# yangbang18/CARE

Hardware: AMD Instinct MI355X
Metric: captions/sec (greedy) (higher is better)
Workload: dtype bf16; 1 GPU; MSRVTT Transformer/base task=Base feats=ViT modality=ami greedy (BASELINE.json configs[1]): [B,28,128]+[B,28,2048]+[B,28,512] fp32 feats, d=512, V=10547, 29 decoder steps; config_name=msrvtt_base_ami, global_batch=32768, lanes=1, parallelism=batch-sharded dp1 (no data-path collective; all-gather of results), hip_graph=True, absorbed_cross_attention=True, lean_encode=True

## Files before the change

care_amd/csrc/gemm_ln.hip:

```cpp
#include <cstdlib>
#include <type_traits>

#include "care_common.h"

namespace {

constexpr int LN_N = 512;

struct LnArgs {
  const void* A; int64_t lda;
  const bf16_t* W;
  const float* bias; const float* res; int64_t ldres; const float* pos;
  const float* gamma; const float* beta; float eps;
  float* out; bf16_t* outb; int64_t ldo;
  int M, K, grp, out_grp_rows, out_row_off;
  int w_packed;
};

template <int N>
__device__ __forceinline__ void ln_wait_vm() {
  if constexpr (N == 5) asm volatile("s_waitcnt vmcnt(5)" ::: "memory");
  else if constexpr (N == 6) asm volatile("s_waitcnt vmcnt(6)" ::: "memory");
  else if constexpr (N == 9) asm volatile("s_waitcnt vmcnt(9)" ::: "memory");
  else if constexpr (N == 10) asm volatile("s_waitcnt vmcnt(10)" ::: "memory");
  else asm volatile("s_waitcnt vmcnt(0)" ::: "memory");
}

template <bool AF32, int RG>
__global__ __launch_bounds__(256 * RG, RG == 1 ? 1 : 2) void gemm_ln_kernel(LnArgs p) {
  constexpr int BM = 64 * RG, NW = 4 * RG;
  constexpr int A_ROWB = AF32 ? 128 : 64;
  constexpr int A_BYTES = BM * A_ROWB, W_BYTES = LN_N * 64, SLOT = A_BYTES + W_BYTES;
  constexpr int NA = A_BYTES / 1024, NWI = W_BYTES / 1024;
  constexpr int NPW = (NA + NWI) / NW;
  static_assert((NA + NWI) % NW == 0, "DMA instructions must divide evenly over the waves");
  extern __shared__ __attribute__((aligned(16))) unsigned char smem[];

  const int tid = threadIdx.x, lane = tid & 63;
  const int wave = __builtin_amdgcn_readfirstlane(tid >> 6);
  const int rg = wave >> 2, cg = wave & 3;
  const int fr = lane & 15, fg = lane >> 4;
  const int m0 = blockIdx.x * BM;
  constexpr unsigned HTAB = (2u) | (3u << 3) | (4u << 6) | (2u << 9) | (5u << 12) | (7u << 15) | (4u << 18) | (1u << 21);

  const unsigned char* src[NPW];
  int dst_off[NPW];
#pragma unroll
  for (int i = 0; i < NPW; ++i) {
    const int q = wave * NPW + i;
    if (q < NA) {
      if constexpr (AF32) {
        const int row = q * 8 + (lane >> 3), pch = lane & 7;
        const int ch = pch ^ ((HTAB >> (3 * ((row & 15) >> 1))) & 7);
        const int grow = min(m0 + row, p.M - 1);
        src[i] = reinterpret_cast<const unsigned char*>(reinterpret_cast<const float*>(p.A) + (int64_t)grow * p.lda) + ch * 16;
      } else {
        const int row = q * 16 + (lane >> 2), pch = lane & 3;
        const int ch = pch ^ ((row & 8) >> 2);
        const int grow = min(m0 + row, p.M - 1);
        src[i] = reinterpret_cast<const unsigned char*>(reinterpret_cast<const bf16_t*>(p.A) + (int64_t)grow * p.lda) + ch * 16;
      }
      dst_off[i] = q * 1024;
    } else {
      const int n = (q - NA) * 16 + (lane >> 2), pch = lane & 3;
      const int ch = pch ^ ((n & 8) >> 2);
      src[i] = reinterpret_cast<const unsigned char*>(p.W + (int64_t)n * p.K) + ch * 16;
      dst_off[i] = A_BYTES + (q - NA) * 1024;
    }
  }
  auto stage = [&](int kt, int slot) {
#pragma unroll
    for (int i = 0; i < NPW; ++i) {
      const int q = wave * NPW + i;
      const int step = (q < NA) ? A_ROWB : 64;
      __builtin_amdgcn_global_load_lds((const __attribute__((address_space(1))) void*)(src[i] + (int64_t)kt * step),
                                       (__attribute__((address_space(3))) void*)(smem + slot * SLOT + dst_off[i]),
                                       16, 0, 0);
    }
  };

  f32x4 acc[4][8];
#pragma unroll
  for (int mt = 0; mt < 4; ++mt)
#pragma unroll
    for (int nt = 0; nt < 8; ++nt) acc[mt][nt] = f32x4{0.f, 0.f, 0.f, 0.f};

  int a_off[4][AF32 ? 2 : 1], w_off[8];
#pragma unroll
  for (int mt = 0; mt < 4; ++mt) {
    const int row = rg * 64 + mt * 16 + fr;
    if constexpr (AF32) {
      const int x = (HTAB >> (3 * (fr >> 1))) & 7;
      a_off[mt][0] = row * 128 + (((2 * fg) ^ x) << 4);
      a_off[mt][1] = row * 128 + (((2 * fg + 1) ^ x) << 4);
    } else {
      a_off[mt][0] = row * 64 + ((fg ^ ((fr & 8) >> 2)) << 4);
    }
  }
#pragma unroll
  for (int nt = 0; nt < 8; ++nt) w_off[nt] = A_BYTES + (cg * 128 + nt * 16 + fr) * 64 + ((fg ^ ((fr & 8) >> 2)) << 4);

  const int nk = p.K >> 5;
  stage(0, 0);
  if (nk > 1) stage(1, 1);
  __builtin_amdgcn_sched_barrier(0);

  for (int kt = 0; kt < nk; ++kt) {
    if (kt + 1 < nk) ln_wait_vm<NPW>(); else ln_wait_vm<0>();
    __builtin_amdgcn_s_barrier();
    __builtin_amdgcn_sched_barrier(0);
    if (kt + 2 < nk) stage(kt + 2, (kt + 2) % 3);
    __builtin_amdgcn_sched_barrier(0);
    const unsigned char* sl = smem + (kt % 3) * SLOT;
    bf16x8 fa[4], fb[8];
#pragma unroll
    for (int nt = 0; nt < 8; ++nt) fb[nt] = *reinterpret_cast<const bf16x8*>(sl + w_off[nt]);
#pragma unroll
    for (int mt = 0; mt < 4; ++mt) {
      if constexpr (AF32) {
        const float4 lo = *reinterpret_cast<const float4*>(sl + a_off[mt][0]);
        const float4 hi = *reinterpret_cast<const float4*>(sl + a_off[mt][1]);
        fa[mt][0] = (bf16_t)lo.x; fa[mt][1] = (bf16_t)lo.y; fa[mt][2] = (bf16_t)lo.z; fa[mt][3] = (bf16_t)lo.w;
        fa[mt][4] = (bf16_t)hi.x; fa[mt][5] = (bf16_t)hi.y; fa[mt][6] = (bf16_t)hi.z; fa[mt][7] = (bf16_t)hi.w;
      } else {
        fa[mt] = *reinterpret_cast<const bf16x8*>(sl + a_off[mt][0]);
      }
    }
#pragma unroll
    for (int mt = 0; mt < 4; ++mt)
#pragma unroll
      for (int nt = 0; nt < 8; ++nt)
        acc[mt][nt] = care_mfma_16x16x32_h16(fb[nt], fa[mt], acc[mt][nt], 0, 0, 0);
  }

  float* tile = reinterpret_cast<float*>(smem);
  float4 gm[2], bt[2], bs[2];
#pragma unroll
  for (int h = 0; h < 2; ++h) {
    const int col = (h * 64 + lane) * 4;
    gm[h] = *reinterpret_cast<const float4*>(p.gamma + col);
    bt[h] = *reinterpret_cast<const float4*>(p.beta + col);
    bs[h] = p.bias ? *reinterpret_cast<const float4*>(p.bias + col) : make_float4(0.f, 0.f, 0.f, 0.f);
  }
#pragma unroll 1
  for (int g = 0; g < RG; ++g) {
    __syncthreads();
    if (rg == g) {
#pragma unroll
      for (int mt = 0; mt < 4; ++mt)
#pragma unroll
        for (int nt = 0; nt < 8; ++nt) {
          const int row = mt * 16 + fr;
          const int chunk = (cg * 32 + nt * 4 + fg) ^ fr;
          *reinterpret_cast<f32x4*>(tile + row * LN_N + chunk * 4) = acc[mt][nt];
        }
    }
    __syncthreads();
    constexpr int UNR = 4, RPW = 64 / NW;
#pragma unroll 1
    for (int rb = 0; rb < RPW; rb += UNR) {
      float4 v[UNR][2], rs[UNR][2], ps[UNR][2];
      int grow[UNR];
#pragma unroll
      for (int u = 0; u < UNR; ++u) {
        const int r = wave * RPW + rb + u;
        grow[u] = m0 + g * 64 + r;
        const int gc = min(grow[u], p.M - 1);
#pragma unroll
        for (int h = 0; h < 2; ++h) {
          const int chunk = h * 64 + lane;
          v[u][h] = *reinterpret_cast<const float4*>(tile + r * LN_N + ((chunk ^ (r & 15)) * 4));
          if (p.res) rs[u][h] = *reinterpret_cast<const float4*>(p.res + (int64_t)gc * p.ldres + chunk * 4);
          if (p.pos) ps[u][h] = *reinterpret_cast<const float4*>(p.pos + (int64_t)(gc % p.grp) * LN_N + chunk * 4);
        }
      }
#pragma unroll
      for (int u = 0; u < UNR; ++u) {
        if (grow[u] >= p.M) continue;
#pragma unroll
        for (int h = 0; h < 2; ++h) {
          v[u][h].x += bs[h].x; v[u][h].y += bs[h].y; v[u][h].z += bs[h].z; v[u][h].w += bs[h].w;
          if (p.res) { v[u][h].x += rs[u][h].x; v[u][h].y += rs[u][h].y; v[u][h].z += rs[u][h].z; v[u][h].w += rs[u][h].w; }
          if (p.pos) { v[u][h].x += ps[u][h].x; v[u][h].y += ps[u][h].y; v[u][h].z += ps[u][h].z; v[u][h].w += ps[u][h].w; }
        }
        const float s = ((v[u][0].x + v[u][0].y) + (v[u][0].z + v[u][0].w)) + ((v[u][1].x + v[u][1].y) + (v[u][1].z + v[u][1].w));
        const float mean = care_wave_sum(s) * (1.0f / LN_N);
        float q = 0.f;
#pragma unroll
        for (int h = 0; h < 2; ++h) {
          const float a = v[u][h].x - mean, b = v[u][h].y - mean, c = v[u][h].z - mean, e = v[u][h].w - mean;
          q += (a * a + b * b) + (c * c + e * e);
        }
        const float rstd = 1.0f / sqrtf(care_wave_sum(q) * (1.0f / LN_N) + p.eps);
        const int64_t orow = (int64_t)(grow[u] / p.grp) * p.out_grp_rows + p.out_row_off + (grow[u] % p.grp);
#pragma unroll
        for (int h = 0; h < 2; ++h) {
          const int col = (h * 64 + lane) * 4;
          float4 o;
          o.x = (v[u][h].x - mean) * rstd * gm[h].x + bt[h].x;
          o.y = (v[u][h].y - mean) * rstd * gm[h].y + bt[h].y;
          o.z = (v[u][h].z - mean) * rstd * gm[h].z + bt[h].z;
          o.w = (v[u][h].w - mean) * rstd * gm[h].w + bt[h].w;
          if (p.out) *reinterpret_cast<float4*>(p.out + orow * p.ldo + col) = o;
          if (p.outb) {
            bf16x4 ob;
            ob[0] = (bf16_t)o.x; ob[1] = (bf16_t)o.y; ob[2] = (bf16_t)o.z; ob[3] = (bf16_t)o.w;
            *reinterpret_cast<bf16x4*>(p.outb + orow * p.ldo + col) = ob;
          }
        }
      }
    }
  }
}

template <bool AF32, int RG>
int launch_ln(const LnArgs& p, hipStream_t st) {
  constexpr int BM = 64 * RG;
  constexpr size_t ring = 3 * (BM * (AF32 ? 128 : 64) + LN_N * 64);
  constexpr size_t lds = ring > 64 * LN_N * 4 ? ring : 64 * LN_N * 4;
  const int blocks = (p.M + BM - 1) / BM;
  static std::atomic<unsigned long long> lds_ok{0};
  if (const int e = care_allow_dynamic_lds(reinterpret_cast<const void*>(&gemm_ln_kernel<AF32, RG>), (int)lds, lds_ok)) return e;
  hipLaunchKernelGGL((gemm_ln_kernel<AF32, RG>), dim3(blocks), dim3(256 * RG), lds, st, p);
  return care_launch_status();
}


#ifndef CARE_LN_ST_NT
#define CARE_LN_ST_NT 0
#endif
#ifndef CARE_LN_A_AUX
#define CARE_LN_A_AUX 0
#endif
#ifndef CARE_LN_DBG
#define CARE_LN_DBG 0
#endif
template <bool F16>
__device__ __forceinline__ f32x4 ln2_mfma(const bf16x8& b, const bf16x8& a, const f32x4& c) {
  if constexpr (F16) {
    typedef _Float16 f16x8 __attribute__((ext_vector_type(8)));
    return __builtin_amdgcn_mfma_f32_16x16x32_f16(__builtin_bit_cast(f16x8, b), __builtin_bit_cast(f16x8, a), c, 0, 0, 0);
  } else {
    return care_mfma_16x16x32_h16(b, a, c, 0, 0, 0);
  }
}

template <int N>
__device__ __forceinline__ void ln2_wait_vm() {
  static_assert(N >= 0 && N <= 63, "vmcnt immediate");
  asm volatile("s_waitcnt vmcnt(%0)" ::"n"(N) : "memory");
}

template <int PER, int MAXY>
__device__ __forceinline__ void ln2_wait_stages(int younger) {
  static_assert(MAXY * PER <= 63, "vmcnt range");
  if constexpr (MAXY >= 6) { if (younger >= 6) { ln2_wait_vm<6 * PER>(); return; } }
  if constexpr (MAXY >= 5) { if (younger == 5) { ln2_wait_vm<5 * PER>(); return; } }
  if constexpr (MAXY >= 4) { if (younger == 4) { ln2_wait_vm<4 * PER>(); return; } }
  if constexpr (MAXY >= 3) { if (younger == 3) { ln2_wait_vm<3 * PER>(); return; } }
  if constexpr (MAXY >= 2) { if (younger == 2) { ln2_wait_vm<2 * PER>(); return; } }
  if constexpr (MAXY >= 1) { if (younger == 1) { ln2_wait_vm<PER>(); return; } }
  ln2_wait_vm<0>();
}

template <bool AF32, int RG, int NSW, int NSA, int EPI, int REP = 1>
__global__ __launch_bounds__(256 * RG, RG) void gemm_ln2_kernel(LnArgs p) {
  static_assert(REP == 1 || (REP == 3 && AF32), "split products need the fp32 operand");
  constexpr int BM = 64 * RG, NW = 4 * RG, NLD = NW / 2;
  constexpr int A_ROWB = 256, KSUB = AF32 ? 2 : 4;
  constexpr int A_BYTES = BM * A_ROWB, W_BYTES = LN_N * 64;
  constexpr int A_BASE = NSW * W_BYTES;
  constexpr int NWI = W_BYTES / 1024 / NLD;
  constexpr int NAI = A_BYTES / 1024 / NLD;
  static_assert(NSW >= 2 && NSA >= 2, "ring depths");
  constexpr bool AE = NSA == 2;
  static_assert(!AE || (!AF32 && REP == 1), "early A issue: bf16 A only");
  extern __shared__ __attribute__((aligned(16))) unsigned char smem[];

  const int tid = threadIdx.x, lane = tid & 63;
  const int wave = __builtin_amdgcn_readfirstlane(tid >> 6);
  const int rg = wave >> 2, cg = wave & 3;
  const int fr = lane & 15, fg = lane >> 4;
  const int m0 = blockIdx.x * BM;
  const bool w_loader = wave < NLD;
  constexpr unsigned HTAB = (2u) | (3u << 3) | (4u << 6) | (2u << 9) | (5u << 12) | (7u << 15) | (4u << 18) | (1u << 21);

  const unsigned w_lane = p.w_packed ? (unsigned)lane * 16u
                                     : (unsigned)(lane >> 2) * (unsigned)p.K * 2u + (unsigned)(((lane & 3) ^ (((lane >> 2) & 8) >> 2)) << 4);
  unsigned a_src[NAI];
#pragma unroll
  for (int i = 0; i < NAI; ++i) {
    const int row = ((w_loader ? 0 : wave - NLD) * NAI + i) * 4 + (lane >> 4);
    const int ch = (lane & 15) ^ (row & 15);
    a_src[i] = (unsigned)(min(m0 + row, p.M - 1) - m0) * (unsigned)p.lda * (AF32 ? 4u : 2u) + (unsigned)ch * 16u;
  }
  const unsigned char* a_blk = reinterpret_cast<const unsigned char*>(p.A) + (int64_t)m0 * p.lda * (AF32 ? 4 : 2);
  auto dma_w = [&](int kt, int slot, int i) {
    if (CARE_LN_DBG & 2) return;
    const int q = wave * NWI + i;
    const unsigned char* base = reinterpret_cast<const unsigned char*>(p.W) +
                                (p.w_packed ? (int64_t)kt * W_BYTES + q * 1024 : (int64_t)(q * 16) * p.K * 2 + (int64_t)kt * 64);
    __builtin_amdgcn_global_load_lds((const __attribute__((address_space(1))) void*)(base + w_lane),
                                     (__attribute__((address_space(3))) void*)(smem + (slot % NSW) * W_BYTES + q * 1024),
                                     16, 0, 0);
  };
  auto dma_a = [&](int m, int slot, int i) {
    if (CARE_LN_DBG & 4) return;
    __builtin_amdgcn_global_load_lds((const __attribute__((address_space(1))) void*)(a_blk + (int64_t)m * A_ROWB + a_src[i]),
                                     (__attribute__((address_space(3))) void*)(smem + A_BASE + (slot % NSA) * A_BYTES + ((wave - NLD) * NAI + i) * 1024),
                                     16, 0, CARE_LN_A_AUX);
  };

  f32x4 acc[4][8];
#pragma unroll
  for (int mt = 0; mt < 4; ++mt)
#pragma unroll
    for (int nt = 0; nt < 8; ++nt) acc[mt][nt] = f32x4{0.f, 0.f, 0.f, 0.f};

  const int w_off0 = (cg * 128 + 8 * (fr >> 2) + (fr & 3)) * 64 + ((fg ^ ((fr & 4) >> 1)) << 4);
  const int a_lane = A_BASE + (rg * 64 + fr) * A_ROWB + (((AF32 ? 2 * fg : fg) ^ fr) << 4);
  auto read_b = [&](int kt, int h, bf16x8 (&f)[4]) {
    if (CARE_LN_DBG & 8) { for (int q = 0; q < 4; ++q) { f[q] = bf16x8{}; asm volatile("" : "+v"(f[q])); } return; }
    const unsigned char* sw = smem + (kt % NSW) * W_BYTES + w_off0;
#pragma unroll
    for (int q = 0; q < 4; ++q) {
      const int nt = h * 4 + q;
      f[q] = *reinterpret_cast<const bf16x8*>(sw + ((nt >> 1) * 32 + (nt & 1) * 4) * 64);
    }
  };
  using araw_t = typename std::conditional<AF32, f32x4, bf16x8>::type;
  auto read_a = [&](int kt, int part, araw_t (&r)[2][AF32 ? 2 : 1]) {
    if (CARE_LN_DBG & 8) { for (int t = 0; t < 2; ++t) for (int c = 0; c < (AF32 ? 2 : 1); ++c) { r[t][c] = araw_t{}; asm volatile("" : "+v"(r[t][c])); } return; }
    const int kr = kt / REP;
    const int jx = (kr % KSUB) * (AF32 ? 128 : 64);
    const unsigned char* sa = smem + ((kr / KSUB) % NSA) * A_BYTES + (a_lane ^ jx);
    const unsigned char* sx = smem + ((kr / KSUB) % NSA) * A_BYTES + (a_lane ^ jx ^ 16);
#pragma unroll
    for (int t = 0; t < 2; ++t) {
      r[t][0] = *reinterpret_cast<const araw_t*>(sa + (2 * part + t) * 16 * A_ROWB);
      if constexpr (AF32) r[t][1] = *reinterpret_cast<const araw_t*>(sx + (2 * part + t) * 16 * A_ROWB);
    }
  };
  auto cvt_a = [&](const araw_t (&r)[2][AF32 ? 2 : 1], bf16x8 (&f)[4], int part, int kt) {
    const bool lo = REP == 3 && kt % REP == 2;
#pragma unroll
    for (int t = 0; t < 2; ++t) {
      if constexpr (AF32) {
        typedef float f32x2 __attribute__((ext_vector_type(2)));
        typedef h16_t bf16x2 __attribute__((ext_vector_type(2)));
        if constexpr (REP == 3) {
          typedef _Float16 f16x2 __attribute__((ext_vector_type(2)));
          typedef unsigned u32x4v __attribute__((ext_vector_type(4)));
          u32x4v packed;
#pragma unroll
          for (int c = 0; c < 2; ++c)
#pragma unroll
            for (int e = 0; e < 4; e += 2) {
              f16x2 pr = __builtin_convertvector(f32x2{r[t][c][e], r[t][c][e + 1]}, f16x2);
              if (lo) pr = __builtin_convertvector(f32x2{r[t][c][e] - (float)pr[0], r[t][c][e + 1] - (float)pr[1]}, f16x2);
              packed[2 * c + (e >> 1)] = __builtin_bit_cast(unsigned, pr);
            }
          f[2 * part + t] = __builtin_bit_cast(bf16x8, packed);
        } else {
#pragma unroll
          for (int c = 0; c < 2; ++c)
#pragma unroll
            for (int e = 0; e < 4; e += 2) {
              bf16x2 pr = __builtin_convertvector(f32x2{r[t][c][e], r[t][c][e + 1]}, bf16x2);
              f[2 * part + t][4 * c + e] = pr[0]; f[2 * part + t][4 * c + e + 1] = pr[1];
            }
        }
      } else {
        f[2 * part + t] = r[t][0];
      }
    }
  };

  const int nk = (p.K >> 5) * REP, nmac = (p.K >> 5) / KSUB;
  constexpr int NAS = NAI / KSUB;
  static_assert(NAI % KSUB == 0 && 16 % NAI == 0, "A issue schedule");
  if (w_loader) {
#pragma unroll 1
    for (int s = 0; s < NSW; ++s)
#pragma unroll
      for (int i = 0; i < NWI; ++i) dma_w(min(s, nk - 1), s, i);
    ln2_wait_vm<(NSW - 1) * NWI>();
  } else {
#pragma unroll 1
    for (int s = 0; s < NSA - 1; ++s)
#pragma unroll
      for (int i = 0; i < NAI; ++i) dma_a(min(s, nmac - 1), s, i);
    ln2_wait_vm<(NSA - 2) * NAI>();
  }
  __builtin_amdgcn_s_barrier();
  __builtin_amdgcn_sched_barrier(0);

  bf16x8 faA[4], fbA[4], faB[4], fbB[4];
  {
    araw_t r0[2][AF32 ? 2 : 1], r1[2][AF32 ? 2 : 1];
    read_a(0, 0, r0); read_a(0, 1, r1); read_b(0, 0, fbA);
    cvt_a(r0, faA, 0, 0); cvt_a(r1, faA, 1, 0);
  }
  auto kstep = [&](int kt, bf16x8 (&fa)[4], bf16x8 (&fb0)[4], bf16x8 (&fan)[4], bf16x8 (&fbn)[4]) {
    const bool more = kt + 1 < nk;
    const int kr = kt / REP, mode = kt % REP;
    const int mac = kr / KSUB, sub = kr % KSUB;
    const bool a_issue = mode == 0;
    const bool a_edge = sub == KSUB - 1 && mode == REP - 1;
    bf16x8 fb1[4];
    araw_t ra[2][AF32 ? 2 : 1], rb[2][AF32 ? 2 : 1];
    __builtin_amdgcn_sched_barrier(0);
    read_b(kt, 1, fb1);
    __builtin_amdgcn_sched_barrier(0);
#pragma unroll
    for (int mt = 0; mt < 4; ++mt)
#pragma unroll
      for (int q = 0; q < 4; ++q)
        if (CARE_LN_DBG & 1) asm volatile("" :: "v"(fb0[q]), "v"(fa[mt]));
        else acc[mt][q] = ln2_mfma<REP == 3>(fb0[q], fa[mt], acc[mt][q]);
    __builtin_amdgcn_sched_barrier(0);
    if (more) {
      if (w_loader) ln2_wait_vm<(NSW - 2) * NWI>();
      else if (a_edge) ln2_wait_vm<AE ? 0 : REP == 1 ? (NSA - 3) * NAI + (KSUB - 1) * NAS : (NSA - 2) * NAI>();
      asm volatile("s_waitcnt lgkmcnt(0)" ::: "memory");
      __builtin_amdgcn_s_barrier();
      __builtin_amdgcn_sched_barrier(0);
      read_a(kt + 1, 0, ra);
      read_b(kt + 1, 0, fbn);
    }
    __builtin_amdgcn_sched_barrier(0);
    const int wst = min(kt + NSW, nk - 1), wslot = kt + NSW;
    const int ast = min(mac - 1 + NSA, nmac - 1), aslot = mac - 1 + NSA;
#pragma unroll
    for (int mt = 0; mt < 4; ++mt) {
#pragma unroll
      for (int q = 0; q < 4; ++q) {
        if (CARE_LN_DBG & 1) asm volatile("" :: "v"(fb1[q]), "v"(fa[mt]));
        else acc[mt][4 + q] = ln2_mfma<REP == 3>(fb1[q], fa[mt], acc[mt][4 + q]);
        const int m = mt * 4 + q;
        if ((m + 1) % (16 / NWI) == 0 || (m + 1) % (16 / (AE ? NAI : NAS)) == 0) {
          if (w_loader) { if ((m + 1) % (16 / NWI) == 0) dma_w(wst, wslot, m / (16 / NWI)); }
          else if (AE) { if (sub == 0 && (m + 1) % (16 / NAI) == 0) dma_a(ast, aslot, m / (16 / NAI)); }
          else { if (a_issue && (m + 1) % (16 / NAS) == 0) dma_a(ast, aslot, sub * NAS + m / (16 / NAS)); }
        }
        __builtin_amdgcn_sched_barrier(0);
      }
      if (mt == 1 && more) {
        cvt_a(ra, fan, 0, kt + 1);
        read_a(kt + 1, 1, rb);
        __builtin_amdgcn_sched_barrier(0);
      }
    }
    if (more) cvt_a(rb, fan, 1, kt + 1);
  };

#pragma unroll 1
  for (int kt = 0; kt < nk; kt += 2) {
    kstep(kt, faA, fbA, faB, fbB);
    kstep(kt + 1, faB, fbB, faA, fbA);
  }

  asm volatile("s_waitcnt vmcnt(0) lgkmcnt(0)" ::: "memory");
  __builtin_amdgcn_s_barrier();
  if (CARE_LN_DBG & 16) {
    float s = 0.f;
#pragma unroll
    for (int mt = 0; mt < 4; ++mt)
#pragma unroll
      for (int nt = 0; nt < 8; ++nt) s += acc[mt][nt][0] + acc[mt][nt][1] + acc[mt][nt][2] + acc[mt][nt][3];
    if (s == 12345.678f && p.outb) p.outb[0] = (bf16_t)s;
    return;
  }
  float* stat = reinterpret_cast<float*>(smem);
  const int col0 = cg * 128 + 8 * fg;
  int m0e = m0;
  asm volatile("" : "+s"(m0e));
  int grow[4];
#pragma unroll
  for (int mt = 0; mt < 4; ++mt) grow[mt] = m0e + rg * 64 + mt * 16 + fr;

  float rsum[4] = {0.f, 0.f, 0.f, 0.f};
  {
    int dep = 0;
    int64_t roff[4], poff[4];
#pragma unroll
    for (int mt = 0; mt < 4; ++mt) {
      const int gc = min(grow[mt], p.M - 1);
      roff[mt] = (int64_t)gc * p.ldres;
      poff[mt] = (int64_t)(gc % p.grp) * LN_N;
    }
#pragma unroll
    for (int pq = 0; pq < 4; ++pq) {
      const int c = col0 + 32 * pq;
      float4 b0 = make_float4(0.f, 0.f, 0.f, 0.f), b1 = b0;
      if (p.bias) { b0 = *reinterpret_cast<const float4*>(p.bias + c); b1 = *reinterpret_cast<const float4*>(p.bias + c + 4); }
      float4 r[4][2], q[4][2];
#pragma unroll
      for (int mth = 0; mth < 2; ++mth) {
#pragma unroll
      for (int mt = 2 * mth; mt < 2 * mth + 2; ++mt) {
        if constexpr (EPI == 1) {
          r[mt][0] = *reinterpret_cast<const float4*>(p.res + roff[mt] + c + dep);
          r[mt][1] = *reinterpret_cast<const float4*>(p.res + roff[mt] + c + 4 + dep);
        }
        if constexpr (EPI == 2) {
          q[mt][0] = *reinterpret_cast<const float4*>(p.pos + poff[mt] + c);
          q[mt][1] = *reinterpret_cast<const float4*>(p.pos + poff[mt] + c + 4);
        }
      }
#pragma unroll
      for (int mt = 2 * mth; mt < 2 * mth + 2; ++mt) {
        f32x4& v0 = acc[mt][2 * pq];
        f32x4& v1 = acc[mt][2 * pq + 1];
        v0[0] += b0.x; v0[1] += b0.y; v0[2] += b0.z; v0[3] += b0.w;
        v1[0] += b1.x; v1[1] += b1.y; v1[2] += b1.z; v1[3] += b1.w;
        if constexpr (EPI == 1) {
          v0[0] += r[mt][0].x; v0[1] += r[mt][0].y; v0[2] += r[mt][0].z; v0[3] += r[mt][0].w;
          v1[0] += r[mt][1].x; v1[1] += r[mt][1].y; v1[2] += r[mt][1].z; v1[3] += r[mt][1].w;
        }
        if constexpr (EPI == 2) {
          v0[0] += q[mt][0].x; v0[1] += q[mt][0].y; v0[2] += q[mt][0].z; v0[3] += q[mt][0].w;
          v1[0] += q[mt][1].x; v1[1] += q[mt][1].y; v1[2] += q[mt][1].z; v1[3] += q[mt][1].w;
        }
        rsum[mt] += ((v0[0] + v0[1]) + (v0[2] + v0[3])) + ((v1[0] + v1[1]) + (v1[2] + v1[3]));
      }
      asm volatile("" : "+v"(dep) : "v"(rsum[2 * mth]), "v"(rsum[2 * mth + 1]));
      __builtin_amdgcn_sched_barrier(0);
      }
    }
  }
  float mean[4], rstd[4];
#pragma unroll
  for (int mt = 0; mt < 4; ++mt) {
    float s = rsum[mt];
    s += __shfl_xor(s, 16, 64);
    s += __shfl_xor(s, 32, 64);
    if (fg == 0) stat[(rg * 64 + mt * 16 + fr) * 4 + cg] = s;
  }
  __syncthreads();
#pragma unroll
  for (int mt = 0; mt < 4; ++mt) {
    const float4 t = *reinterpret_cast<const float4*>(stat + (rg * 64 + mt * 16 + fr) * 4);
    mean[mt] = ((t.x + t.y) + (t.z + t.w)) * (1.0f / LN_N);
  }
#pragma unroll
  for (int mt = 0; mt < 4; ++mt) {
    float q = 0.f;
#pragma unroll
    for (int nt = 0; nt < 8; ++nt) {
      const float a = acc[mt][nt][0] - mean[mt], b = acc[mt][nt][1] - mean[mt];
      const float c = acc[mt][nt][2] - mean[mt], e = acc[mt][nt][3] - mean[mt];
      q += (a * a + b * b) + (c * c + e * e);
    }
    q += __shfl_xor(q, 16, 64);
    q += __shfl_xor(q, 32, 64);
    if (fg == 0) stat[BM * 4 + (rg * 64 + mt * 16 + fr) * 4 + cg] = q;
  }
  __syncthreads();
  int64_t orow[4];
#pragma unroll
  for (int mt = 0; mt < 4; ++mt) {
    const float4 t = *reinterpret_cast<const float4*>(stat + BM * 4 + (rg * 64 + mt * 16 + fr) * 4);
    rstd[mt] = 1.0f / sqrtf(((t.x + t.y) + (t.z + t.w)) * (1.0f / LN_N) + p.eps);
    orow[mt] = (int64_t)(grow[mt] / p.grp) * p.out_grp_rows + p.out_row_off + (grow[mt] % p.grp);
  }
  const float* gam = p.gamma;
  const float* bet = p.beta;
  asm volatile("" : "+s"(gam), "+s"(bet));
#pragma unroll
  for (int pq = 0; pq < 4; ++pq) {
    const int c = col0 + 32 * pq;
    const float4 g0 = *reinterpret_cast<const float4*>(gam + c), g1 = *reinterpret_cast<const float4*>(gam + c + 4);
    const float4 e0 = *reinterpret_cast<const float4*>(bet + c), e1 = *reinterpret_cast<const float4*>(bet + c + 4);
#pragma unroll
    for (int mt = 0; mt < 4; ++mt) {
      if (grow[mt] >= p.M) continue;
      const f32x4 v0 = acc[mt][2 * pq], v1 = acc[mt][2 * pq + 1];
      float4 o0, o1;
      o0.x = (v0[0] - mean[mt]) * rstd[mt] * g0.x + e0.x; o0.y = (v0[1] - mean[mt]) * rstd[mt] * g0.y + e0.y;
      o0.z = (v0[2] - mean[mt]) * rstd[mt] * g0.z + e0.z; o0.w = (v0[3] - mean[mt]) * rstd[mt] * g0.w + e0.w;
      o1.x = (v1[0] - mean[mt]) * rstd[mt] * g1.x + e1.x; o1.y = (v1[1] - mean[mt]) * rstd[mt] * g1.y + e1.y;
      o1.z = (v1[2] - mean[mt]) * rstd[mt] * g1.z + e1.z; o1.w = (v1[3] - mean[mt]) * rstd[mt] * g1.w + e1.w;
      if (CARE_LN_DBG & 32) { if (o0.x + o0.y + o0.z + o0.w + o1.x + o1.y + o1.z + o1.w != 12345.678f) continue; }
      if (p.out) {
        float* op = p.out + orow[mt] * p.ldo + c;
        *reinterpret_cast<float4*>(op) = o0;
        *reinterpret_cast<float4*>(op + 4) = o1;
      }
      if (p.outb) {
        bf16x8 ob;
        ob[0] = (bf16_t)o0.x; ob[1] = (bf16_t)o0.y; ob[2] = (bf16_t)o0.z; ob[3] = (bf16_t)o0.w;
        ob[4] = (bf16_t)o1.x; ob[5] = (bf16_t)o1.y; ob[6] = (bf16_t)o1.z; ob[7] = (bf16_t)o1.w;
        if (CARE_LN_ST_NT) __builtin_nontemporal_store(ob, reinterpret_cast<bf16x8*>(p.outb + orow[mt] * p.ldo + c));
        else *reinterpret_cast<bf16x8*>(p.outb + orow[mt] * p.ldo + c) = ob;
      }
    }
  }
}

template <bool AF32, int RG, int NSW, int NSA, int EPI, int REP = 1>
int launch_ln2e(const LnArgs& p, hipStream_t st) {
  constexpr int BM = 64 * RG;
  constexpr int LDS = NSW * LN_N * 64 + NSA * BM * 256;
  static_assert(LDS <= 160 * 1024, "LDS budget");
  static std::atomic<unsigned long long> lds_ok{0};
  if (const int e = care_allow_dynamic_lds(reinterpret_cast<const void*>(&gemm_ln2_kernel<AF32, RG, NSW, NSA, EPI, REP>), LDS, lds_ok)) return e;
  hipLaunchKernelGGL((gemm_ln2_kernel<AF32, RG, NSW, NSA, EPI, REP>), dim3((p.M + BM - 1) / BM), dim3(256 * RG), LDS, st, p);
  return care_launch_status();
}

template <bool AF32, int RG, int NSW, int NSA>
int launch_ln2(const LnArgs& p, hipStream_t st) {
  if (p.res) return launch_ln2e<AF32, RG, NSW, NSA, 1>(p, st);
  return launch_ln2e<AF32, RG, NSW, NSA, 0>(p, st);
}

constexpr int WS_NSW = 3, WS_NSA = 2;
constexpr int LN3_MIN_BLOCKS = 8;
constexpr int WS_W_BYTES = LN_N * 64;
constexpr int WS_A_BYTES = 128 * 128;
constexpr int WS_A_BASE = WS_NSW * WS_W_BYTES;
constexpr int WS_STAT = WS_A_BASE + WS_NSA * WS_A_BYTES;
constexpr int WS_PAR = WS_STAT + 2 * 128 * 4 * 4;
constexpr int WS_LDS = WS_PAR + 3 * LN_N * 4;
#ifndef CARE_LN3_DBG
#define CARE_LN3_DBG 0
#endif
#ifndef CARE_LN3_A_NT
#define CARE_LN3_A_NT 1
#endif

template <bool OUT32>
__global__ __launch_bounds__(768) void gemm_ln3_kernel(LnArgs p) {
  extern __shared__ __attribute__((aligned(16))) unsigned char smem[];
  const int tid = threadIdx.x, lane = tid & 63;
  const int wave = __builtin_amdgcn_readfirstlane(tid >> 6);
  const int nk = p.K >> 5, nmac = nk >> 1;
  const int nblk = (p.M + 127) >> 7;
  const int mine = (nblk - (int)blockIdx.x + (int)gridDim.x - 1) / (int)gridDim.x;
  const int total = mine * nk, total_mac = mine * nmac;
  auto stamp = [&](int g, int k) {
    if (!(CARE_LN3_DBG & 64) || blockIdx.x != 0 || g >= 256 || lane != 0) return;
    reinterpret_cast<unsigned long long*>(p.out)[(wave * 256 + g) * 4 + k] = __builtin_amdgcn_s_memtime();
  };

  if (wave >= 10) {
    const int al = wave - 10, q4 = lane >> 4, c16 = lane & 15;
    const int64_t ldab = p.lda * 4;
    const unsigned voff = (unsigned)q4 * (unsigned)ldab + (unsigned)c16 * 16u;
    const int lw = (64 * al + q4) * 128 + ((((c16 >> 1) ^ (q4 >> 1)) << 4) | ((c16 & 1) << 3));
    f32x4 R0[16], R1[16];
    int lbi = 0, lmac = 0;
    const unsigned char* lrow = reinterpret_cast<const unsigned char*>(p.A) + ((int64_t)blockIdx.x * 128 + 64 * al) * ldab;
    auto load_half = [&](f32x4 (&R)[16], int h) {
#pragma unroll
      for (int i = 8 * h; i < 8 * h + 8; ++i) {
        const unsigned char* base = lrow + (int64_t)(4 * i) * ldab + (int64_t)lmac * 256;
        if (CARE_LN3_DBG & 4) { asm volatile("" : "+v"(R[i])); continue; }
        if (CARE_LN3_A_NT) asm volatile("global_load_dwordx4 %0, %1, %2 nt\n\ts_nop 0" : "+v"(R[i]) : "v"(voff), "s"(base) : "memory");
        else asm volatile("global_load_dwordx4 %0, %1, %2\n\ts_nop 0" : "+v"(R[i]) : "v"(voff), "s"(base) : "memory");
      }
      if (h == 1 && ++lmac == nmac) {
        if (lbi + 1 < mine) { lmac = 0; ++lbi; lrow += (int64_t)gridDim.x * 128 * ldab; }
        else lmac = nmac - 1;
      }
    };
    auto landed = [&](f32x4 (&R)[16], int h, bool steady) {
      if (steady) asm volatile("s_waitcnt vmcnt(24)" : "+v"(R[8 * h]), "+v"(R[8 * h + 1]), "+v"(R[8 * h + 2]), "+v"(R[8 * h + 3]), "+v"(R[8 * h + 4]), "+v"(R[8 * h + 5]), "+v"(R[8 * h + 6]), "+v"(R[8 * h + 7])::"memory");
      else asm volatile("s_waitcnt vmcnt(0)" : "+v"(R[8 * h]), "+v"(R[8 * h + 1]), "+v"(R[8 * h + 2]), "+v"(R[8 * h + 3]), "+v"(R[8 * h + 4]), "+v"(R[8 * h + 5]), "+v"(R[8 * h + 6]), "+v"(R[8 * h + 7])::"memory");
    };
    auto store_half = [&](int m, f32x4 (&R)[16], int h) {
      unsigned char* dst = smem + WS_A_BASE + (m & 1) * WS_A_BYTES;
      typedef float f32x2 __attribute__((ext_vector_type(2)));
      typedef h16_t hx2 __attribute__((ext_vector_type(2)));
#pragma unroll
      for (int i = 8 * h; i < 8 * h + 8; ++i) {
        const hx2 lo = __builtin_convertvector(f32x2{R[i][0], R[i][1]}, hx2), hi = __builtin_convertvector(f32x2{R[i][2], R[i][3]}, hx2);
        bf16x4 o;
        o[0] = lo[0]; o[1] = lo[1]; o[2] = hi[0]; o[3] = hi[1];
        *reinterpret_cast<bf16x4*>(dst + i * 512 + (lw ^ (((2 * i) & 7) << 4))) = o;
      }
    };
    auto produce = [&](int m, f32x4 (&R)[16], int h) {
      landed(R, h, true);
      store_half(m + 1, R, h);
      __builtin_amdgcn_sched_barrier(0);
      load_half(R, h);
      asm volatile("s_waitcnt lgkmcnt(0)" ::: "memory");
    };
#pragma unroll
    for (int i = 0; i < 16; ++i) { R0[i] = f32x4{0.f, 0.f, 0.f, 0.f}; R1[i] = R0[i]; }
    load_half(R0, 0); load_half(R0, 1);
    load_half(R1, 0); load_half(R1, 1);
    landed(R0, 0, false); landed(R0, 1, false);
    store_half(0, R0, 0); store_half(0, R0, 1);
    __builtin_amdgcn_sched_barrier(0);
    load_half(R0, 0); load_half(R0, 1);
    asm volatile("s_waitcnt lgkmcnt(0)" ::: "memory");
    __builtin_amdgcn_s_barrier();
    auto period = [&](int m, f32x4 (&R)[16]) {
      stamp(2 * m, 0);
      produce(m, R, 0);
      stamp(2 * m, 1);
      if (m > 0 && m % nmac == 0) { __builtin_amdgcn_s_barrier(); __builtin_amdgcn_s_barrier(); }
      __builtin_amdgcn_s_barrier();
      stamp(2 * m + 1, 0);
      produce(m, R, 1);
      stamp(2 * m + 1, 1);
      __builtin_amdgcn_s_barrier();
    };
#pragma unroll 1
    for (int m = 0; m < total_mac; m += 2) {
      period(m, R1);
      period(m + 1, R0);
    }
    __builtin_amdgcn_s_barrier(); __builtin_amdgcn_s_barrier();
    return;
  }

  if (wave >= 8) {
    const int wl = wave - 8;
    const unsigned char* wsrc = reinterpret_cast<const unsigned char*>(p.W) + wl * 16384 + lane * 16;
    int ikt = 0, islot = 0, issued = 0;
    auto issue = [&]() {
      const unsigned char* s = wsrc + (int64_t)ikt * WS_W_BYTES;
      unsigned char* d = smem + islot * WS_W_BYTES + wl * 16384;
#pragma unroll
      for (int i = 0; i < 16; ++i)
        if (!(CARE_LN3_DBG & 2)) __builtin_amdgcn_global_load_lds((const __attribute__((address_space(1))) void*)(s + i * 1024),
                                         (__attribute__((address_space(3))) void*)(d + i * 1024), 16, 0, 0);
      ikt = ikt + 1 == nk ? 0 : ikt + 1;
      islot = islot + 1 == WS_NSW ? 0 : islot + 1;
      ++issued;
    };
    while (issued < min(WS_NSW - 1, total)) issue();
    if (issued > 1) ln2_wait_vm<16>(); else ln2_wait_vm<0>();
    __builtin_amdgcn_s_barrier();
    int kt = 0;
#pragma unroll 1
    for (int g = 0; g < total; ++g) {
      stamp(g, 0);
      if (issued < min(g + WS_NSW, total)) issue();
      stamp(g, 1);
      if (g > 0 && kt == 0) { __builtin_amdgcn_s_barrier(); __builtin_amdgcn_s_barrier(); }
      if (issued > g + 2) ln2_wait_vm<16>(); else ln2_wait_vm<0>();
      stamp(g, 2);
      __builtin_amdgcn_s_barrier();
      stamp(g, 3);
      kt = kt + 1 == nk ? 0 : kt + 1;
    }
    __builtin_amdgcn_s_barrier(); __builtin_amdgcn_s_barrier();
    return;
  }

  const int rg = wave >> 2, cg = wave & 3;
  const int fr = lane & 15, fg = lane >> 4;
  const int w_off0 = (cg * 128 + 8 * (fr >> 2) + (fr & 3)) * 64 + ((fg ^ ((fr & 4) >> 1)) << 4);
  const int a_lane = WS_A_BASE + (rg * 64 + fr) * 128 + ((fg ^ ((fr >> 1) & 7)) << 4);
  float* stat = reinterpret_cast<float*>(smem + WS_STAT);
  const float* par = reinterpret_cast<const float*>(smem + WS_PAR);
  for (int i = tid; i < 3 * LN_N; i += 512)
    reinterpret_cast<float*>(smem + WS_PAR)[i] = i < LN_N ? (p.bias ? p.bias[i] : 0.f) : i < 2 * LN_N ? p.gamma[i - LN_N] : p.beta[i - 2 * LN_N];
  asm volatile("s_waitcnt lgkmcnt(0)" ::: "memory");
  __builtin_amdgcn_s_barrier();
  int wslot = 0, g = 0;
#pragma unroll 1
  for (int bi = 0; bi < mine; ++bi) {
    f32x4 acc[4][8];
#pragma unroll
    for (int mt = 0; mt < 4; ++mt)
#pragma unroll
      for (int nt = 0; nt < 8; ++nt) acc[mt][nt] = f32x4{0.f, 0.f, 0.f, 0.f};
#pragma unroll 1
    for (int kt = 0; kt < nk; ++kt, ++g) {
      const unsigned char* sw = smem + wslot * WS_W_BYTES + w_off0;
      const unsigned char* sa = smem + ((g >> 1) & 1) * WS_A_BYTES + (a_lane ^ ((g & 1) << 6));
      bf16x8 fa[4], fb[2][2];
      stamp(g, 0);
      auto rd = [&](const unsigned char* q) {
        if (CARE_LN3_DBG & 8) { bf16x8 z = {}; asm volatile("" : "+v"(z)); return z; }
        return *reinterpret_cast<const bf16x8*>(q);
      };
#pragma unroll
      for (int mt = 0; mt < 4; ++mt) fa[mt] = rd(sa + mt * 16 * 128);
      fb[0][0] = rd(sw);
      fb[0][1] = rd(sw + 4 * 64);
#pragma unroll
      for (int pr = 0; pr < 4; ++pr) {
        if (pr < 3) {
          fb[(pr + 1) & 1][0] = rd(sw + (pr + 1) * 32 * 64);
          fb[(pr + 1) & 1][1] = rd(sw + ((pr + 1) * 32 + 4) * 64);
        }
        __builtin_amdgcn_sched_barrier(0);
#pragma unroll
        for (int mt = 0; mt < 4; ++mt) {
          if (CARE_LN3_DBG & 1) { asm volatile("" :: "v"(fb[pr & 1][0]), "v"(fb[pr & 1][1]), "v"(fa[mt])); continue; }
          acc[mt][2 * pr] = care_mfma_16x16x32_h16(fb[pr & 1][0], fa[mt], acc[mt][2 * pr], 0, 0, 0);
          acc[mt][2 * pr + 1] = care_mfma_16x16x32_h16(fb[pr & 1][1], fa[mt], acc[mt][2 * pr + 1], 0, 0, 0);
        }
      }
      wslot = wslot + 1 == WS_NSW ? 0 : wslot + 1;
      stamp(g, 1);
      __builtin_amdgcn_sched_barrier(0);
      asm volatile("s_waitcnt lgkmcnt(0)" ::: "memory");
      __builtin_amdgcn_s_barrier();
      __builtin_amdgcn_sched_barrier(0);
    }

    const int m0 = ((int)blockIdx.x + bi * (int)gridDim.x) * 128;
    if (CARE_LN3_DBG & 16) {
      float s = 0.f;
#pragma unroll
      for (int mt = 0; mt < 4; ++mt)
#pragma unroll
        for (int nt = 0; nt < 8; ++nt) s += acc[mt][nt][0] + acc[mt][nt][1] + acc[mt][nt][2] + acc[mt][nt][3];
      if (s == 12345.678f && p.outb) p.outb[0] = (bf16_t)s;
      __builtin_amdgcn_s_barrier(); __builtin_amdgcn_s_barrier();
      continue;
    }
    int lid, grp = p.grp;
    asm volatile("v_mbcnt_lo_u32_b32 %0, -1, 0\n\tv_mbcnt_hi_u32_b32 %0, -1, %0" : "=v"(lid));
    asm volatile("" : "+s"(grp));
    const int fre = lid & 15, fge = lid >> 4;
    auto xlane = [&](float v, int mask) { return __builtin_bit_cast(float, __builtin_amdgcn_ds_bpermute((lid ^ mask) << 2, __builtin_bit_cast(int, v))); };
    const int col0e = cg * 128 + 8 * fge;
    const int srow = (rg * 64 + fre) * 4;
    float rsum[4] = {0.f, 0.f, 0.f, 0.f};
#pragma unroll
    for (int pq = 0; pq < 4; ++pq) {
      const f32x4 b0 = *reinterpret_cast<const f32x4*>(par + col0e + 32 * pq), b1 = *reinterpret_cast<const f32x4*>(par + col0e + 32 * pq + 4);
#pragma unroll
      for (int mt = 0; mt < 4; ++mt) {
        f32x4& v0 = acc[mt][2 * pq];
        f32x4& v1 = acc[mt][2 * pq + 1];
        v0 += b0; v1 += b1;
        rsum[mt] += ((v0[0] + v0[1]) + (v0[2] + v0[3])) + ((v1[0] + v1[1]) + (v1[2] + v1[3]));
      }
    }
#pragma unroll
    for (int mt = 0; mt < 4; ++mt) {
      float s = rsum[mt];
      s += xlane(s, 16);
      s += xlane(s, 32);
      if (fge == 0) stat[srow + mt * 64 + cg] = s;
    }
    __syncthreads();
#pragma unroll
    for (int mt = 0; mt < 4; ++mt) {
      const float4 t = *reinterpret_cast<const float4*>(stat + srow + mt * 64);
      const float mean = ((t.x + t.y) + (t.z + t.w)) * (1.0f / LN_N);
      float q = 0.f;
#pragma unroll
      for (int nt = 0; nt < 8; ++nt) {
        acc[mt][nt] -= mean;
        const float a = acc[mt][nt][0], b = acc[mt][nt][1], c = acc[mt][nt][2], e = acc[mt][nt][3];
        q += (a * a + b * b) + (c * c + e * e);
      }
      q += xlane(q, 16);
      q += xlane(q, 32);
      if (fge == 0) stat[128 * 4 + srow + mt * 64 + cg] = q;
    }
    __syncthreads();
    int orow[4];
#pragma unroll
    for (int mt = 0; mt < 4; ++mt) {
      const float4 t = *reinterpret_cast<const float4*>(stat + 128 * 4 + srow + mt * 64);
      const float rstd = 1.0f / sqrtf(((t.x + t.y) + (t.z + t.w)) * (1.0f / LN_N) + p.eps);
#pragma unroll
      for (int nt = 0; nt < 8; ++nt) acc[mt][nt] *= rstd;
      const int grow = m0 + rg * 64 + mt * 16 + fre;
      orow[mt] = (grow / grp) * p.out_grp_rows + p.out_row_off + (grow % grp);
    }
#pragma unroll
    for (int pq = 0; pq < 4; ++pq) {
      const int c = col0e + 32 * pq;
      typedef h16_t hx4 __attribute__((ext_vector_type(4)));
      hx4 h0[4];
      {
        const f32x4 g0 = *reinterpret_cast<const f32x4*>(par + LN_N + c), e0 = *reinterpret_cast<const f32x4*>(par + 2 * LN_N + c);
#pragma unroll
        for (int mt = 0; mt < 4; ++mt) {
          const f32x4 o = acc[mt][2 * pq] * g0 + e0;
          if (OUT32 && !(CARE_LN3_DBG & 96)) *reinterpret_cast<f32x4*>(p.out + (int64_t)orow[mt] * p.ldo + c) = o;
          h0[mt] = hx4{(h16_t)o[0], (h16_t)o[1], (h16_t)o[2], (h16_t)o[3]};
        }
      }
      const f32x4 g1 = *reinterpret_cast<const f32x4*>(par + LN_N + c + 4), e1 = *reinterpret_cast<const f32x4*>(par + 2 * LN_N + c + 4);
#pragma unroll
      for (int mt = 0; mt < 4; ++mt) {
        const f32x4 o = acc[mt][2 * pq + 1] * g1 + e1;
        if (OUT32 && !(CARE_LN3_DBG & 96)) *reinterpret_cast<f32x4*>(p.out + (int64_t)orow[mt] * p.ldo + c + 4) = o;
        if (CARE_LN3_DBG & 32) { if (o[0] + o[1] + o[2] + o[3] != 12345.678f) continue; }
        if (p.outb) {
          bf16x8 ob;
          ob[0] = h0[mt][0]; ob[1] = h0[mt][1]; ob[2] = h0[mt][2]; ob[3] = h0[mt][3];
          ob[4] = (h16_t)o[0]; ob[5] = (h16_t)o[1]; ob[6] = (h16_t)o[2]; ob[7] = (h16_t)o[3];
          *reinterpret_cast<bf16x8*>(p.outb + (int64_t)orow[mt] * p.ldo + c) = ob;
        }
      }
    }
    stamp(g - 1, 2);
  }
}

int launch_ln3(const LnArgs& p, hipStream_t st) {
  static std::atomic<unsigned long long> lds_ok{0};
  static std::atomic<unsigned long long> lds_ok32{0};
  const bool out32 = p.out != nullptr && !(CARE_LN3_DBG & 64);
  if (const int e = out32 ? care_allow_dynamic_lds(reinterpret_cast<const void*>(&gemm_ln3_kernel<true>), WS_LDS, lds_ok32)
                          : care_allow_dynamic_lds(reinterpret_cast<const void*>(&gemm_ln3_kernel<false>), WS_LDS, lds_ok)) return e;
  static const int cus = [] {
    int dev = 0, n = 0;
    if (hipGetDevice(&dev) != hipSuccess || hipDeviceGetAttribute(&n, hipDeviceAttributeMultiprocessorCount, dev) != hipSuccess || n < 1) n = 256;
    return n;
  }();
  const int nblk = (p.M + 127) / 128;
// ... 413 lines not shown
```

Before: 669,700 captions/s.

## Stream LayerNorm residual and bias through LDS via async global-to-LDS loads

Adds an RL variant of the fused GEMM+LayerNorm epilogue. Each wave DMAs its residual rows (double-buffered 16-row tiles, XOR-swizzled) and the bias into LDS with global_load_lds, then reads them with ds_read_b128 while adding them to the accumulators. This replaces scattered per-lane float4 global loads of the residual and overlaps those loads with the epilogue arithmetic. It is on by default for aligned residuals, can be disabled with CARE_LN_RES_LDS=0, and adds LDS traffic and inline-asm complexity.

```diff
diff --git a/care_amd/csrc/gemm_ln.hip b/care_amd/csrc/gemm_ln.hip
--- a/care_amd/csrc/gemm_ln.hip
+++ b/care_amd/csrc/gemm_ln.hip
@@ -263,9 +263,11 @@
   ln2_wait_vm<0>();
 }
 
-template <bool AF32, int RG, int NSW, int NSA, int EPI, int REP = 1>
+constexpr int LN2_RES_WAVE = 2 * 16 * 512 + 1024;
+template <bool AF32, int RG, int NSW, int NSA, int EPI, int REP = 1, bool RL = false>
 __global__ __launch_bounds__(256 * RG, RG) void gemm_ln2_kernel(LnArgs p) {
   static_assert(REP == 1 || (REP == 3 && AF32), "split products need the fp32 operand");
+  static_assert(!RL || EPI == 1, "only a residual travels through LDS");
   constexpr int BM = 64 * RG, NW = 4 * RG, NLD = NW / 2;
   constexpr int A_ROWB = 256, KSUB = AF32 ? 2 : 4;
   constexpr int A_BYTES = BM * A_ROWB, W_BYTES = LN_N * 64;
@@ -310,6 +312,7 @@
                                      (__attribute__((address_space(3))) void*)(smem + A_BASE + (slot % NSA) * A_BYTES + ((wave - NLD) * NAI + i) * 1024),
                                      16, 0, CARE_LN_A_AUX);
   };
+  const int nk = (p.K >> 5) * REP, nmac = (p.K >> 5) / KSUB;
 
   f32x4 acc[4][8];
 #pragma unroll
@@ -376,7 +379,6 @@
     }
   };
 
-  const int nk = (p.K >> 5) * REP, nmac = (p.K >> 5) / KSUB;
   constexpr int NAS = NAI / KSUB;
   static_assert(NAI % KSUB == 0 && 16 % NAI == 0, "A issue schedule");
   if (w_loader) {
@@ -471,7 +473,7 @@
     if (s == 12345.678f && p.outb) p.outb[0] = (bf16_t)s;
     return;
   }
-  float* stat = reinterpret_cast<float*>(smem);
+  float* stat = reinterpret_cast<float*>(smem + (RL ? NW * LN2_RES_WAVE : 0));
   const int col0 = cg * 128 + 8 * fg;
   int m0e = m0;
   asm volatile("" : "+s"(m0e));
@@ -480,7 +482,77 @@
   for (int mt = 0; mt < 4; ++mt) grow[mt] = m0e + rg * 64 + mt * 16 + fr;
 
   float rsum[4] = {0.f, 0.f, 0.f, 0.f};
-  {
+  if constexpr (RL) {
+    constexpr int TILE_B = 16 * 512, NTI = TILE_B / 1024;
+    static_assert(LN2_RES_WAVE == 2 * TILE_B + 1024 && NW * LN2_RES_WAVE + 2 * BM * 4 * 4 <= NSW * W_BYTES + NSA * A_BYTES, "residual regions + statistics exchange");
+    const int wbase = wave * LN2_RES_WAVE;
+    const float* bia = p.bias;
+    asm volatile("" : "+s"(bia));
+    int lanee = lane;
+    asm volatile("" : "+v"(lanee));
+    if (bia) {
+      __builtin_amdgcn_global_load_lds((const __attribute__((address_space(1))) void*)(reinterpret_cast<const unsigned char*>(bia) + cg * 512 + (unsigned)((lanee & 31) << 4)),
+                                       (__attribute__((address_space(3))) void*)(smem + wbase + 2 * TILE_B), 16, 0, 0);
+    } else {
+      reinterpret_cast<float4*>(smem + wbase + 2 * TILE_B)[lanee] = make_float4(0.f, 0.f, 0.f, 0.f);
+    }
+    auto issue_tile = [&](int mt) {
+      if (CARE_LN_DBG & 64) return;
+#pragma unroll
+      for (int i = 0; i < NTI; ++i) {
+        const int r = 2 * i + (lanee >> 5);
+        const int64_t off = (int64_t)min(m0e + rg * 64 + mt * 16 + r, p.M - 1) * p.ldres * 4 + cg * 512 + (((lanee & 31) ^ r) << 4);
+        __builtin_amdgcn_global_load_lds((const __attribute__((address_space(1))) void*)(reinterpret_cast<const unsigned char*>(p.res) + off),
+                                         (__attribute__((address_space(3))) void*)(smem + wbase + (mt & 1) * TILE_B + i * 1024), 16, 0, 0);
+      }
+    };
+    const unsigned lbase = (unsigned)(uintptr_t)(__attribute__((address_space(3))) unsigned char*)smem + (unsigned)wbase;
+    const unsigned bb = lbase + (unsigned)(2 * TILE_B + ((lanee >> 4) & 3) * 32);
+    float prev = 0.f;
+    unsigned rd[4];
+#pragma unroll
+    for (int x = 0; x < 4; ++x)
+      rd[x] = lbase + (unsigned)((lanee & 15) * 512 + ((((x >> 1) * 8 + ((lanee >> 4) & 3) * 2 + (x & 1)) ^ (lanee & 15)) << 4));
+    issue_tile(0);
+    issue_tile(1);
+#pragma unroll
+    for (int mt = 0; mt < 4; ++mt) {
+      if (mt < 3 && !(CARE_LN_DBG & 64)) ln2_wait_vm<NTI>(); else ln2_wait_vm<0>();
+#pragma unroll
+      for (int hp = 0; hp < 2; ++hp) {
+        const unsigned o = (unsigned)((mt & 1) * TILE_B + hp * 256);
+        const unsigned a0 = rd[0] + o, a1 = rd[1] + o, a2 = rd[2] + o, a3 = rd[3] + o, ab = bb + hp * 256;
+        f32x4 r[2][2], b[2][2];
+        asm volatile(
+            "ds_read_b128 %0, %8\n\t"
+            "ds_read_b128 %1, %8 offset:16\n\t"
+            "ds_read_b128 %2, %8 offset:128\n\t"
+            "ds_read_b128 %3, %8 offset:144\n\t"
+            "ds_read_b128 %4, %9\n\t"
+            "ds_read_b128 %5, %10\n\t"
+            "ds_read_b128 %6, %11\n\t"
+            "ds_read_b128 %7, %12\n\t"
+            "s_waitcnt lgkmcnt(0)"
+            : "=&v"(b[0][0]), "=&v"(b[0][1]), "=&v"(b[1][0]), "=&v"(b[1][1]), "=&v"(r[0][0]), "=&v"(r[0][1]), "=&v"(r[1][0]), "=&v"(r[1][1])
+            : "v"(ab), "v"(a0), "v"(a1), "v"(a2), "v"(a3), "v"(prev)
+            : "memory");
+        if (hp == 1 && mt < 2) issue_tile(mt + 2);
+#pragma unroll
+        for (int k = 0; k < 2; ++k) {
+          const int pq = 2 * hp + k;
+          f32x4& v0 = acc[mt][2 * pq];
+          f32x4& v1 = acc[mt][2 * pq + 1];
+          v0[0] += b[k][0][0]; v0[1] += b[k][0][1]; v0[2] += b[k][0][2]; v0[3] += b[k][0][3];
+          v1[0] += b[k][1][0]; v1[1] += b[k][1][1]; v1[2] += b[k][1][2]; v1[3] += b[k][1][3];
+          v0[0] += r[k][0][0]; v0[1] += r[k][0][1]; v0[2] += r[k][0][2]; v0[3] += r[k][0][3];
+          v1[0] += r[k][1][0]; v1[1] += r[k][1][1]; v1[2] += r[k][1][2]; v1[3] += r[k][1][3];
+          rsum[mt] += ((v0[0] + v0[1]) + (v0[2] + v0[3])) + ((v1[0] + v1[1]) + (v1[2] + v1[3]));
+        }
+        prev = rsum[mt];
+        __builtin_amdgcn_sched_barrier(0);
+      }
+    }
+  } else {
     int dep = 0;
     int64_t roff[4], poff[4];
 #pragma unroll
@@ -500,8 +572,12 @@
 #pragma unroll
       for (int mt = 2 * mth; mt < 2 * mth + 2; ++mt) {
         if constexpr (EPI == 1) {
-          r[mt][0] = *reinterpret_cast<const float4*>(p.res + roff[mt] + c + dep);
-          r[mt][1] = *reinterpret_cast<const float4*>(p.res + roff[mt] + c + 4 + dep);
+          if (CARE_LN_DBG & 64) {
+            r[mt][0] = r[mt][1] = make_float4(0.f, 0.f, 0.f, 0.f);
+          } else {
+            r[mt][0] = *reinterpret_cast<const float4*>(p.res + roff[mt] + c + dep);
+            r[mt][1] = *reinterpret_cast<const float4*>(p.res + roff[mt] + c + 4 + dep);
+          }
         }
         if constexpr (EPI == 2) {
           q[mt][0] = *reinterpret_cast<const float4*>(p.pos + poff[mt] + c);
@@ -598,20 +674,24 @@
   }
 }
 
-template <bool AF32, int RG, int NSW, int NSA, int EPI, int REP = 1>
+template <bool AF32, int RG, int NSW, int NSA, int EPI, int REP = 1, bool RL = false>
 int launch_ln2e(const LnArgs& p, hipStream_t st) {
   constexpr int BM = 64 * RG;
   constexpr int LDS = NSW * LN_N * 64 + NSA * BM * 256;
   static_assert(LDS <= 160 * 1024, "LDS budget");
   static std::atomic<unsigned long long> lds_ok{0};
-  if (const int e = care_allow_dynamic_lds(reinterpret_cast<const void*>(&gemm_ln2_kernel<AF32, RG, NSW, NSA, EPI, REP>), LDS, lds_ok)) return e;
-  hipLaunchKernelGGL((gemm_ln2_kernel<AF32, RG, NSW, NSA, EPI, REP>), dim3((p.M + BM - 1) / BM), dim3(256 * RG), LDS, st, p);
+  if (const int e = care_allow_dynamic_lds(reinterpret_cast<const void*>(&gemm_ln2_kernel<AF32, RG, NSW, NSA, EPI, REP, RL>), LDS, lds_ok)) return e;
+  hipLaunchKernelGGL((gemm_ln2_kernel<AF32, RG, NSW, NSA, EPI, REP, RL>), dim3((p.M + BM - 1) / BM), dim3(256 * RG), LDS, st, p);
   return care_launch_status();
 }
 
 template <bool AF32, int RG, int NSW, int NSA>
 int launch_ln2(const LnArgs& p, hipStream_t st) {
-  if (p.res) return launch_ln2e<AF32, RG, NSW, NSA, 1>(p, st);
+  if (p.res) {
+    const char* rl = getenv("CARE_LN_RES_LDS");
+    if ((!rl || atoi(rl)) && care_aligned16(p.res)) return launch_ln2e<AF32, RG, NSW, NSA, 1, 1, true>(p, st);
+    return launch_ln2e<AF32, RG, NSW, NSA, 1>(p, st);
+  }
   return launch_ln2e<AF32, RG, NSW, NSA, 0>(p, st);
 }
 
```

After: 649,000 captions/s. 3.1% lower.
